# darrenjkt/SEE-VCN

Measured on AMD Instinct MI355X. Metric: scenes/sec (VCN+voxel+spconv fwd+bwd), higher is better.
Workload: dtype f32; 1 GPU; VCN_VC fwd on 64 objects x 1024 pts -> kNN surface select (k=30) -> largest DBSCAN cluster (eps 0.4) -> unique + replace (<0.1 m) into 16 KITTI-shaped 64-beam scenes (21.0k pts in range each) -> DynMeanVFE -> VoxelBackBone8x + HeightCompression fwd+bwd + SGD (BASELINE configs[1]+[2]); scenes_per_gpu=16, objects_per_gpu=64, points_per_object=1024, geometry=KITTI [0,-40,-3,70.4,40,1] @ [0.05,0.05,0.1] -> sparse [41,1600,1408], parallelism=dp1, input_side=side stream, one batch ahead (every step = 1 front + 1 compute)

## Files before the change

### see-vcn_amd/csrc/norm.h

```cpp
#pragma once
#include "common.h"

#define BN_THREADS 256
#define BN_MAX_C 512
#define BN_MAX_WGS 1024

struct BnArgs {
  const float* x;
  const float* dy;
  float* out;
  const float* gamma;
  const float* beta;
  float* running_mean;
  float* running_var;
  float* save_mean;
  float* save_invstd;
  float* dgamma;
  float* dbeta;
  float* partial;
  float* coef;
  int64_t n;
  int C, relu, wgs;
  float momentum, eps;
  int64_t* num_batches_tracked;
};

__device__ __forceinline__ float bn_shift(float mean, float scale, float beta) { return __fmaf_rn(-mean, scale, beta); }
__device__ __forceinline__ float bn_act(float x, float scale, float shift) { return __fmaf_rn(x, scale, shift); }

void sv_bn_finalize_fwd(const BnArgs& a, hipStream_t st);
void sv_bn_finalize_bwd(const BnArgs& a, hipStream_t st);
```

### see-vcn_amd/csrc/norm.hip

```cpp
#include <string.h>

#include "common.h"

#include "norm.h"

template <bool BWD>
__global__ __launch_bounds__(BN_THREADS) void k_bn_reduce(BnArgs a) {
  __shared__ float s_red[2][BN_THREADS * 4];
  const int tid = threadIdx.x, C4 = a.C >> 2;
  const int R = BN_THREADS / C4;
  const int c4 = tid % C4, rr = tid / C4;
  const bool active = rr < R;
  const int64_t rows_per_wg = (a.n + a.wgs - 1) / a.wgs;
  const int64_t r0 = (int64_t)blockIdx.x * rows_per_wg, r1 = min(a.n, r0 + rows_per_wg);
  float4 s0 = make_float4(0, 0, 0, 0), s1 = make_float4(0, 0, 0, 0);
  float4 mean = make_float4(0, 0, 0, 0), istd = mean, g = make_float4(1, 1, 1, 1), bt = mean;
  if (BWD && active) {
    mean = reinterpret_cast<const float4*>(a.save_mean)[c4], istd = reinterpret_cast<const float4*>(a.save_invstd)[c4];
    if (a.gamma) g = reinterpret_cast<const float4*>(a.gamma)[c4];
    if (a.beta) bt = reinterpret_cast<const float4*>(a.beta)[c4];
  }
  const float4 sc = make_float4(istd.x * g.x, istd.y * g.y, istd.z * g.z, istd.w * g.w);
  const float4 sh = make_float4(bn_shift(mean.x, sc.x, bt.x), bn_shift(mean.y, sc.y, bt.y), bn_shift(mean.z, sc.z, bt.z), bn_shift(mean.w, sc.w, bt.w));
  if (active) {
    for (int64_t r = r0 + rr; r < r1; r += R) {
      const float4 v = reinterpret_cast<const float4*>(a.x + r * a.C)[c4];
      if (!BWD) {
        s0.x += v.x, s0.y += v.y, s0.z += v.z, s0.w += v.w;
        s1.x += v.x * v.x, s1.y += v.y * v.y, s1.z += v.z * v.z, s1.w += v.w * v.w;
      } else {
        float4 d = reinterpret_cast<const float4*>(a.dy + r * a.C)[c4];
        const float4 xh = make_float4((v.x - mean.x) * istd.x, (v.y - mean.y) * istd.y, (v.z - mean.z) * istd.z, (v.w - mean.w) * istd.w);
        if (a.relu) {
          d.x = (bn_act(v.x, sc.x, sh.x) > 0.f) ? d.x : 0.f, d.y = (bn_act(v.y, sc.y, sh.y) > 0.f) ? d.y : 0.f;
          d.z = (bn_act(v.z, sc.z, sh.z) > 0.f) ? d.z : 0.f, d.w = (bn_act(v.w, sc.w, sh.w) > 0.f) ? d.w : 0.f;
        }
        s0.x += d.x, s0.y += d.y, s0.z += d.z, s0.w += d.w;
        s1.x += d.x * xh.x, s1.y += d.y * xh.y, s1.z += d.z * xh.z, s1.w += d.w * xh.w;
      }
    }
  }
  reinterpret_cast<float4*>(s_red[0])[tid] = s0;
  reinterpret_cast<float4*>(s_red[1])[tid] = s1;
  __syncthreads();
  if (tid < C4) {
    float4 t0 = make_float4(0, 0, 0, 0), t1 = t0;
    for (int q = 0; q < R; ++q) {
      const float4 u0 = reinterpret_cast<float4*>(s_red[0])[q * C4 + tid], u1 = reinterpret_cast<float4*>(s_red[1])[q * C4 + tid];
      t0.x += u0.x, t0.y += u0.y, t0.z += u0.z, t0.w += u0.w;
      t1.x += u1.x, t1.y += u1.y, t1.z += u1.z, t1.w += u1.w;
    }
    float* p = a.partial + (size_t)blockIdx.x * 2 * a.C;
    reinterpret_cast<float4*>(p)[tid] = t0;
    reinterpret_cast<float4*>(p + a.C)[tid] = t1;
  }
}

__device__ __forceinline__ void bn_combine(const BnArgs& a, int c, double* s0, double* s1, double& t0, double& t1) {
  const int tid = threadIdx.x;
  t0 = 0.0, t1 = 0.0;
  for (int w = tid; w < a.wgs; w += BN_THREADS) {
    t0 += (double)a.partial[(size_t)w * 2 * a.C + c];
    t1 += (double)a.partial[(size_t)w * 2 * a.C + a.C + c];
  }
  s0[tid] = t0, s1[tid] = t1;
  __syncthreads();
  for (int off = BN_THREADS / 2; off > 0; off >>= 1) {
    if (tid < off) s0[tid] += s0[tid + off], s1[tid] += s1[tid + off];
    __syncthreads();
  }
  t0 = s0[0], t1 = s1[0];
}
__device__ __forceinline__ void bn_finish_fwd(const BnArgs& a, int c, double t0, double t1, double n) {
  const float gm = a.gamma ? a.gamma[c] : 1.f, bb = a.beta ? a.beta[c] : 0.f;
  const double m = t0 / n;
  double var = t1 / n - m * m;
  var = var < 0.0 ? 0.0 : var;
  const float invstd = (float)(1.0 / sqrt(var + (double)a.eps));
  a.save_mean[c] = (float)m, a.save_invstd[c] = invstd;
  if (a.running_mean) {
    const double unbiased = n > 1.0 ? var * n / (n - 1.0) : var;
    a.running_mean[c] = (1.f - a.momentum) * a.running_mean[c] + a.momentum * (float)m;
    a.running_var[c] = (1.f - a.momentum) * a.running_var[c] + a.momentum * (float)unbiased;
  }
  const float scale = invstd * gm;
  a.coef[c] = scale;
  a.coef[a.C + c] = bn_shift((float)m, scale, bb);
}
__device__ __forceinline__ void bn_coef_bwd(const BnArgs& a, int c, double t0, double t1, double n) {
  const float gm = a.gamma ? a.gamma[c] : 1.f;
  const float invstd = a.save_invstd[c], m = a.save_mean[c];
  a.coef[c] = gm * invstd;
  a.coef[a.C + c] = (float)(t0 / n);
  a.coef[2 * a.C + c] = (float)(t1 / n);
  a.coef[3 * a.C + c] = m;
}

template <bool BWD>
__global__ __launch_bounds__(BN_THREADS) void k_bn_finalize(BnArgs a) {
  __shared__ double s0[BN_THREADS], s1[BN_THREADS];
  const int c = blockIdx.x;
  if (!BWD && c == 0 && threadIdx.x == 0 && a.num_batches_tracked) *a.num_batches_tracked += 1;
  double t0, t1;
  bn_combine(a, c, s0, s1, t0, t1);
  if (threadIdx.x != 0) return;
  if (!BWD) {
    bn_finish_fwd(a, c, t0, t1, (double)a.n);
  } else {
    a.dbeta[c] = (float)t0, a.dgamma[c] = (float)t1;
    bn_coef_bwd(a, c, t0, t1, (double)a.n);
  }
}

template <bool BWD>
__global__ __launch_bounds__(BN_THREADS) void k_bn_sums_local(BnArgs a, double* out) {
  __shared__ double s0[BN_THREADS], s1[BN_THREADS];
  const int c = blockIdx.x;
  double t0, t1;
  bn_combine(a, c, s0, s1, t0, t1);
  if (threadIdx.x != 0) return;
  out[c] = t0, out[a.C + c] = t1;
  if (!BWD && c == 0) out[2 * a.C] = (double)a.n;
  if (BWD) a.dbeta[c] = (float)t0, a.dgamma[c] = (float)t1;
}
// ... 5 lines not shown
  for (int r = 1; r < world; ++r) t0 += gathered[r * stride + c], t1 += gathered[r * stride + a.C + c], n += gathered[r * stride + 2 * a.C];
  if (c == 0) {
    if (a.num_batches_tracked) *a.num_batches_tracked += 1;
    if (total_rows) *total_rows = n;
  }
  bn_finish_fwd(a, c, t0, t1, n);
}
__global__ void k_bn_coef_bwd_global(BnArgs a, const double* gathered, int world, const double* total_rows) {
  const int c = blockIdx.x * blockDim.x + threadIdx.x;
  if (c >= a.C) return;
  const size_t stride = 2 * (size_t)a.C;
  double t0 = gathered[c], t1 = gathered[a.C + c];
  for (int r = 1; r < world; ++r) t0 += gathered[r * stride + c], t1 += gathered[r * stride + a.C + c];
  bn_coef_bwd(a, c, t0, t1, *total_rows);
}

__global__ __launch_bounds__(BN_THREADS) void k_bn_apply_fwd(BnArgs a) {
  const int C4 = a.C >> 2;
  const int64_t total = a.n * C4;
  for (int64_t i = (int64_t)blockIdx.x * BN_THREADS + threadIdx.x; i < total; i += (int64_t)gridDim.x * BN_THREADS) {
    const int c4 = (int)(i % C4);
    const float4 v = reinterpret_cast<const float4*>(a.x)[i];
    const float4 sc = reinterpret_cast<const float4*>(a.coef)[c4], sh = reinterpret_cast<const float4*>(a.coef + a.C)[c4];
    float4 y = make_float4(bn_act(v.x, sc.x, sh.x), bn_act(v.y, sc.y, sh.y), bn_act(v.z, sc.z, sh.z), bn_act(v.w, sc.w, sh.w));
    if (a.relu) y.x = fmaxf(y.x, 0.f), y.y = fmaxf(y.y, 0.f), y.z = fmaxf(y.z, 0.f), y.w = fmaxf(y.w, 0.f);
    reinterpret_cast<float4*>(a.out)[i] = y;
  }
}

__global__ __launch_bounds__(BN_THREADS) void k_bn_apply_bwd(BnArgs a) {
  const int C4 = a.C >> 2;
  const int64_t total = a.n * C4;
  for (int64_t i = (int64_t)blockIdx.x * BN_THREADS + threadIdx.x; i < total; i += (int64_t)gridDim.x * BN_THREADS) {
    const int c4 = (int)(i % C4);
    const float4 v = reinterpret_cast<const float4*>(a.x)[i];
    float4 d = reinterpret_cast<const float4*>(a.dy)[i];
    const float4 k = reinterpret_cast<const float4*>(a.coef)[c4], md = reinterpret_cast<const float4*>(a.coef + a.C)[c4];
    const float4 mx = reinterpret_cast<const float4*>(a.coef + 2 * a.C)[c4], m = reinterpret_cast<const float4*>(a.coef + 3 * a.C)[c4];
    const float4 istd = reinterpret_cast<const float4*>(a.save_invstd)[c4];
    const float4 xh = make_float4((v.x - m.x) * istd.x, (v.y - m.y) * istd.y, (v.z - m.z) * istd.z, (v.w - m.w) * istd.w);
    if (a.relu) {
      const float4 g = a.gamma ? reinterpret_cast<const float4*>(a.gamma)[c4] : make_float4(1, 1, 1, 1);
      const float4 bt = a.beta ? reinterpret_cast<const float4*>(a.beta)[c4] : make_float4(0, 0, 0, 0);
      const float4 sc = make_float4(istd.x * g.x, istd.y * g.y, istd.z * g.z, istd.w * g.w);
      const float4 sh = make_float4(bn_shift(m.x, sc.x, bt.x), bn_shift(m.y, sc.y, bt.y), bn_shift(m.z, sc.z, bt.z), bn_shift(m.w, sc.w, bt.w));
      d.x = (bn_act(v.x, sc.x, sh.x) > 0.f) ? d.x : 0.f, d.y = (bn_act(v.y, sc.y, sh.y) > 0.f) ? d.y : 0.f;
      d.z = (bn_act(v.z, sc.z, sh.z) > 0.f) ? d.z : 0.f, d.w = (bn_act(v.w, sc.w, sh.w) > 0.f) ? d.w : 0.f;
    }
    reinterpret_cast<float4*>(a.out)[i] = make_float4(k.x * (d.x - md.x - xh.x * mx.x), k.y * (d.y - md.y - xh.y * mx.y),
                                                      k.z * (d.z - md.z - xh.z * mx.z), k.w * (d.w - md.w - xh.w * mx.w));
  }
}

constexpr int BNF_THREADS = 1024;
__global__ __launch_bounds__(BNF_THREADS) void k_bn_bwd_fused(BnArgs a) {
  __shared__ double s_sum[BNF_THREADS * 4];
  __shared__ __attribute__((aligned(16))) float s_coef[4 * BN_MAX_C];
  const int tid = threadIdx.x, C = a.C, C2 = 2 * C, Q = C2 / 4, G = BNF_THREADS / Q;
  {
    const int q = tid % Q, g = tid / Q;
    double t0 = 0.0, t1 = 0.0, t2 = 0.0, t3 = 0.0;
    if (g < G) {
      for (int w = g; w < a.wgs; w += G) {
        const float4 v = reinterpret_cast<const float4*>(a.partial + (size_t)w * C2)[q];
        t0 += (double)v.x, t1 += (double)v.y, t2 += (double)v.z, t3 += (double)v.w;
      }
      double* d = s_sum + (size_t)g * C2 + 4 * q;
      d[0] = t0, d[1] = t1, d[2] = t2, d[3] = t3;
    }
  }
  __syncthreads();
  if (tid < C) {
    double t0 = 0.0, t1 = 0.0;
    for (int g = 0; g < G; ++g) t0 += s_sum[(size_t)g * C2 + tid], t1 += s_sum[(size_t)g * C2 + C + tid];
    const float gm = a.gamma ? a.gamma[tid] : 1.f;
    const float invstd = a.save_invstd[tid], m = a.save_mean[tid];
    if (blockIdx.x == 0) a.dbeta[tid] = (float)t0, a.dgamma[tid] = (float)t1;
    s_coef[tid] = gm * invstd;
    s_coef[C + tid] = (float)(t0 / (double)a.n);
    s_coef[2 * C + tid] = (float)(t1 / (double)a.n);
    s_coef[3 * C + tid] = m;
  }
  __syncthreads();
  const int C4 = C >> 2;
  const int64_t total = a.n * C4;
  for (int64_t i = (int64_t)blockIdx.x * BNF_THREADS + tid; i < total; i += (int64_t)gridDim.x * BNF_THREADS) {
    const int c4 = (int)(i % C4);
    const float4 v = reinterpret_cast<const float4*>(a.x)[i];
    float4 d = reinterpret_cast<const float4*>(a.dy)[i];
    const float4 k = reinterpret_cast<const float4*>(s_coef)[c4], md = reinterpret_cast<const float4*>(s_coef + C)[c4];
    const float4 mx = reinterpret_cast<const float4*>(s_coef + 2 * C)[c4], m = reinterpret_cast<const float4*>(s_coef + 3 * C)[c4];
    const float4 istd = reinterpret_cast<const float4*>(a.save_invstd)[c4];
    const float4 xh = make_float4((v.x - m.x) * istd.x, (v.y - m.y) * istd.y, (v.z - m.z) * istd.z, (v.w - m.w) * istd.w);
    if (a.relu) {
      const float4 g = a.gamma ? reinterpret_cast<const float4*>(a.gamma)[c4] : make_float4(1, 1, 1, 1);
      const float4 bt = a.beta ? reinterpret_cast<const float4*>(a.beta)[c4] : make_float4(0, 0, 0, 0);
      const float4 sc = make_float4(istd.x * g.x, istd.y * g.y, istd.z * g.z, istd.w * g.w);
      const float4 sh = make_float4(bn_shift(m.x, sc.x, bt.x), bn_shift(m.y, sc.y, bt.y), bn_shift(m.z, sc.z, bt.z), bn_shift(m.w, sc.w, bt.w));
      d.x = (bn_act(v.x, sc.x, sh.x) > 0.f) ? d.x : 0.f, d.y = (bn_act(v.y, sc.y, sh.y) > 0.f) ? d.y : 0.f;
      d.z = (bn_act(v.z, sc.z, sh.z) > 0.f) ? d.z : 0.f, d.w = (bn_act(v.w, sc.w, sh.w) > 0.f) ? d.w : 0.f;
    }
    reinterpret_cast<float4*>(a.out)[i] = make_float4(k.x * (d.x - md.x - xh.x * mx.x), k.y * (d.y - md.y - xh.y * mx.y),
                                                      k.z * (d.z - md.z - xh.z * mx.z), k.w * (d.w - md.w - xh.w * mx.w));
  }
}
static void bn_backward_tail(const BnArgs& a, hipStream_t st) {
  static const int fused = getenv("SEEVCN_BN_BWD_FUSED") ? atoi(getenv("SEEVCN_BN_BWD_FUSED")) : 0;
  const int Q = a.C / 2;
  if (fused && Q >= 1 && BNF_THREADS % Q == 0) {
    const int64_t quads = a.n * (a.C / 4);
    int wgs = (int)((quads + BNF_THREADS * 4 - 1) / (BNF_THREADS * 4));
    if (wgs > 256) wgs = 256;
    if (wgs < 1) wgs = 1;
    hipLaunchKernelGGL(k_bn_bwd_fused, dim3(wgs), dim3(BNF_THREADS), 0, st, a);
    return;
  }
  hipLaunchKernelGGL(k_bn_finalize<true>, dim3(a.C), dim3(BN_THREADS), 0, st, a);
  hipLaunchKernelGGL(k_bn_apply_bwd, dim3(sv_grid_1d(a.n * (a.C / 4), BN_THREADS)), dim3(BN_THREADS), 0, st, a);
}

__device__ __forceinline__ void bn_eval_coef(const float* gamma, const float* beta, const float* running_mean, const float* running_var, float eps,
                                             float* coef, int C, int c) {
  const float invstd = 1.f / sqrtf(running_var[c] + eps);
  const float gm = gamma ? gamma[c] : 1.f, bb = beta ? beta[c] : 0.f;
  coef[c] = invstd * gm;
  coef[C + c] = bb - running_mean[c] * invstd * gm;
}

__global__ void k_bn_eval_coef(BnArgs a) {
  const int c = blockIdx.x * blockDim.x + threadIdx.x;
  if (c >= a.C) return;
  bn_eval_coef(a.gamma, a.beta, a.running_mean, a.running_var, a.eps, a.coef, a.C, c);
}

struct BnEvalCoefJob {
  const float *gamma, *beta, *running_mean, *running_var;
  float* coef;
  int C;
  float eps;
};
constexpr int BN_EVAL_JOBS = 64;
struct BnEvalCoefBatch {
  BnEvalCoefJob j[BN_EVAL_JOBS];
};
static_assert(sizeof(BnEvalCoefBatch) <= 3900, "kernel argument block");

__global__ __launch_bounds__(128) void k_bn_eval_coef_batch(BnEvalCoefBatch b) {
  const BnEvalCoefJob& J = b.j[blockIdx.x];
  for (int c = threadIdx.x; c < J.C; c += 128) bn_eval_coef(J.gamma, J.beta, J.running_mean, J.running_var, J.eps, J.coef, J.C, c);
}

extern "C" int sv_batchnorm_eval_coef_batch(const int64_t* jobs_host, int n_jobs, void* stream) {
  SV_CHECK_ARG(n_jobs >= 0 && (jobs_host || n_jobs == 0), "sv_batchnorm_eval_coef_batch: bad arguments");
  if (n_jobs == 0) return SV_OK;
  for (int q = 0; q < n_jobs; ++q) {
    const int64_t* r = jobs_host + 8 * (size_t)q;
    SV_CHECK_ARG(r[2] && r[3] && r[4], "sv_batchnorm_eval_coef_batch: job %d: null pointer", q);
    SV_CHECK_ARG(r[5] >= 1 && r[5] <= BN_MAX_C, "sv_batchnorm_eval_coef_batch: job %d: 1..%d channels (got %lld)", q, BN_MAX_C, (long long)r[5]);
    SV_CHECK_ARG((uintptr_t)r[4] % 16 == 0, "sv_batchnorm_eval_coef_batch: job %d: coef_out must be 16-byte aligned", q);
  }
  hipStream_t st = sv_stream(stream);
  for (int q0 = 0; q0 < n_jobs; q0 += BN_EVAL_JOBS) {
    BnEvalCoefBatch b;
    const int nb = n_jobs - q0 < BN_EVAL_JOBS ? n_jobs - q0 : BN_EVAL_JOBS;
    for (int q = 0; q < nb; ++q) {
      const int64_t* r = jobs_host + 8 * (size_t)(q0 + q);
      BnEvalCoefJob& J = b.j[q];
      J.gamma = reinterpret_cast<const float*>((uintptr_t)r[0]), J.beta = reinterpret_cast<const float*>((uintptr_t)r[1]);
      J.running_mean = reinterpret_cast<const float*>((uintptr_t)r[2]), J.running_var = reinterpret_cast<const float*>((uintptr_t)r[3]);
      J.coef = reinterpret_cast<float*>((uintptr_t)r[4]);
      double eps;
      memcpy(&eps, &r[6], sizeof eps);
      J.C = (int)r[5], J.eps = (float)eps;
    }
    hipLaunchKernelGGL(k_bn_eval_coef_batch, dim3(nb), dim3(128), 0, st, b);
  }
  SV_LAUNCH_CHECK();
  return SV_OK;
}

static int bn_wgs(int64_t n, int C) {
  const int R = BN_THREADS / (C / 4);
  int64_t w = (n + (int64_t)R * 8 - 1) / ((int64_t)R * 8);
  if (w < 1) w = 1;
  if (w > BN_MAX_WGS) w = BN_MAX_WGS;
  return (int)w;
}

extern "C" size_t sv_batchnorm_scratch_bytes(int channels) {
  return ((size_t)BN_MAX_WGS * 2 * channels + 4 * (size_t)channels) * sizeof(float);
}

static int bn_common_check(const char* who, int64_t n, int C) {
  SV_CHECK_ARG(n >= 1, "%s: needs at least one row (got %ld)", who, (long)n);
  SV_CHECK_ARG(C >= 4 && C <= BN_MAX_C && (C & 3) == 0 && BN_THREADS % (C / 4) == 0,
               "%s: channels must be a multiple of 4 with C/4 dividing %d, <= %d (got %d)", who, BN_THREADS, BN_MAX_C, C);
  return SV_OK;
}

static void bn_scratch(BnArgs& a, void* scratch) {
  a.coef = reinterpret_cast<float*>(scratch);
  a.partial = a.coef + 4 * (size_t)a.C;
}

extern "C" int sv_batchnorm_relu_forward(const float* x, int64_t n, int channels, const float* gamma, const float* beta,
                                         float* running_mean, float* running_var, float momentum, float eps, int training, int relu,
                                         void* scratch, float* y, float* save_mean, float* save_invstd, int64_t* num_batches_tracked,
                                         void* stream) {
  if (int rc = bn_common_check("sv_batchnorm_relu_forward", n, channels)) return rc;
  SV_CHECK_ARG(x && y && scratch, "sv_batchnorm_relu_forward: null pointer");
  SV_CHECK_ARG(training ? (save_mean && save_invstd) : (running_mean && running_var),
               "sv_batchnorm_relu_forward: training needs save_mean/save_invstd, eval needs running statistics");
  BnArgs a{};
  a.x = x, a.out = y, a.gamma = gamma, a.beta = beta, a.running_mean = running_mean, a.running_var = running_var;
  a.save_mean = save_mean, a.save_invstd = save_invstd, a.n = n, a.C = channels, a.relu = relu, a.momentum = momentum, a.eps = eps;
  a.wgs = bn_wgs(n, channels);
  a.num_batches_tracked = training ? num_batches_tracked : nullptr;
  bn_scratch(a, scratch);
  hipStream_t st = sv_stream(stream);
  if (training) {
    hipLaunchKernelGGL(k_bn_reduce<false>, dim3(a.wgs), dim3(BN_THREADS), 0, st, a);
    hipLaunchKernelGGL(k_bn_finalize<false>, dim3(channels), dim3(BN_THREADS), 0, st, a);
  } else
    hipLaunchKernelGGL(k_bn_eval_coef, dim3(sv_div_up(channels, 128)), dim3(128), 0, st, a);
  hipLaunchKernelGGL(k_bn_apply_fwd, dim3(sv_grid_1d(n * (channels / 4), BN_THREADS)), dim3(BN_THREADS), 0, st, a);
  SV_LAUNCH_CHECK();
  return SV_OK;
}

extern "C" int sv_batchnorm_relu_forward_partial(const float* x, int64_t n, int channels, const float* gamma, const float* beta, float* running_mean,
                                                 float* running_var, float momentum, float eps, int relu, void* scratch, int n_partials, float* y,
                                                 float* save_mean, float* save_invstd, int64_t* num_batches_tracked, void* stream) {
  if (int rc = bn_common_check("sv_batchnorm_relu_forward_partial", n, channels)) return rc;
  SV_CHECK_ARG(x && y && scratch && save_mean && save_invstd, "sv_batchnorm_relu_forward_partial: null pointer");
  SV_CHECK_ARG(n_partials >= 1 && n_partials <= BN_MAX_WGS, "sv_batchnorm_relu_forward_partial: 1..%d partials (got %d)", BN_MAX_WGS, n_partials);
  BnArgs a{};
  a.x = x, a.out = y, a.gamma = gamma, a.beta = beta, a.running_mean = running_mean, a.running_var = running_var;
  a.save_mean = save_mean, a.save_invstd = save_invstd, a.n = n, a.C = channels, a.relu = relu, a.momentum = momentum, a.eps = eps;
  a.wgs = n_partials;
  a.num_batches_tracked = num_batches_tracked;
  bn_scratch(a, scratch);
  hipStream_t st = sv_stream(stream);
  hipLaunchKernelGGL(k_bn_finalize<false>, dim3(channels), dim3(BN_THREADS), 0, st, a);
// ... 144 lines not shown
```

### see-vcn_amd/csrc/set_abstraction_train.hip

```cpp
#include "norm.h"

typedef float st_f4 __attribute__((ext_vector_type(4)));

constexpr int ST_THREADS = 512;
constexpr int ST_WAVES = ST_THREADS / 64;
constexpr int ST_MAXC = 64;
constexpr int ST_NT = ST_MAXC / 16;
constexpr int ST_MAXF = 128;

constexpr int ST_PITCH = ST_MAXC + 4;
constexpr int ST_GRID = 512;

struct SaT {
  const float* xyz;
  const float* feat;
  const float* new_xyz;
  const int32_t* idx;
  const int32_t* row_start;
  const float* w1;
  const float* w2;
  float* z1;
  float* z2;
  float* dy1;
  float* part;
// ... 7 lines not shown
  float* zmin;
  uint8_t* amax;
  uint8_t* amin;
  float* out;
  const float* dout;
  float* wpart;
  float* S;
  float* P;
  int64_t M, N;
  int C, Kp, C1, C2, ns;
};

__device__ __forceinline__ st_f4 mfma4(const st_f4 a, const st_f4 b, st_f4 c) {
  c = __builtin_amdgcn_mfma_f32_16x16x4f32(a.x, b.x, c, 0, 0, 0);
  c = __builtin_amdgcn_mfma_f32_16x16x4f32(a.y, b.y, c, 0, 0, 0);
  c = __builtin_amdgcn_mfma_f32_16x16x4f32(a.z, b.z, c, 0, 0, 0);
  c = __builtin_amdgcn_mfma_f32_16x16x4f32(a.w, b.w, c, 0, 0, 0);
  return c;
}

__device__ __forceinline__ void tile_to_global(const float* T, float* dst, int C, int lane) {
  const int c4n = C >> 2, nf = 16 * c4n;
  for (int f = lane; f < nf; f += 64) {
    const int row = f / c4n, c4 = f - row * c4n;
    reinterpret_cast<st_f4*>(dst)[f] = *reinterpret_cast<const st_f4*>(T + row * ST_PITCH + c4 * 4);
  }
}

__device__ __forceinline__ void acc_to_lds(float* T, const st_f4 (&acc)[ST_NT], int nt, int li, int kk) {
#pragma unroll
  for (int t = 0; t < ST_NT; ++t)
    if (t < nt) {
#pragma unroll
      for (int r = 0; r < 4; ++r) T[(kk * 4 + r) * ST_PITCH + t * 16 + li] = acc[t][r];
    }
}

__device__ __forceinline__ void stats_to_partial(float (&s0)[ST_NT], float (&s1)[ST_NT], int nt, int C, float (*s_red)[2][ST_MAXC], float* part, int wid,
                                                 int lane) {
  const int li = lane & 15, kk = lane >> 4;
#pragma unroll
  for (int t = 0; t < ST_NT; ++t)
    if (t < nt) {
      float a = s0[t], b = s1[t];
      a += __shfl_xor(a, 16), b += __shfl_xor(b, 16);
      a += __shfl_xor(a, 32), b += __shfl_xor(b, 32);
      if (kk == 0) s_red[wid][0][t * 16 + li] = a, s_red[wid][1][t * 16 + li] = b;
    }
  __syncthreads();
  for (int e = threadIdx.x; e < 2 * C; e += ST_THREADS) {
    const int which = e / C, c = e - which * C;
    float v = 0.f;
    for (int w = 0; w < ST_WAVES; ++w) v += s_red[w][which][c];
    part[(size_t)blockIdx.x * 2 * C + which * C + c] = v;
  }
}

constexpr int SP_THREADS = 256;
__global__ __launch_bounds__(SP_THREADS) void k_sa_point_proj(SaT a) {
  __shared__ __attribute__((aligned(16))) float s_w[ST_MAXC * (ST_MAXF + 4)];
  __shared__ __attribute__((aligned(16))) float s_t[SP_THREADS / 64][16 * ST_PITCH];
  const int tid = threadIdx.x, lane = tid & 63, wid = tid >> 6, li = lane & 15, kk = lane >> 4;
  const int pw = a.C + 4, cin = a.C + 3;
  for (int e = tid; e < a.C1 * a.C; e += SP_THREADS) s_w[(e / a.C) * pw + e % a.C] = a.w1[(e / a.C) * cin + 3 + e % a.C];
  __syncthreads();
  float* T = s_t[wid];
  const int nt1 = a.C1 / 16, nqf = a.C / 16;
  const int64_t ntiles = (a.N + 15) / 16;
  for (int64_t tile = (int64_t)blockIdx.x * (SP_THREADS / 64) + wid; tile < ntiles; tile += (int64_t)gridDim.x * (SP_THREADS / 64)) {
    const int64_t n = tile * 16 + li;
    st_f4 acc[ST_NT];
#pragma unroll
    for (int t = 0; t < ST_NT; ++t) acc[t] = (st_f4){0.f, 0.f, 0.f, 0.f};
    for (int qs = 0; qs < nqf; ++qs) {
      st_f4 A = (st_f4){0.f, 0.f, 0.f, 0.f};
      if (n < a.N) A = *reinterpret_cast<const st_f4*>(a.feat + n * a.C + qs * 16 + kk * 4);
#pragma unroll
      for (int t = 0; t < ST_NT; ++t)
        if (t < nt1) acc[t] = mfma4(A, *reinterpret_cast<const st_f4*>(s_w + (t * 16 + li) * pw + qs * 16 + kk * 4), acc[t]);
    }
    acc_to_lds(T, acc, nt1, li, kk);
    __builtin_amdgcn_fence(__ATOMIC_RELEASE, "wavefront");
    const int rows = (int)min((int64_t)16, a.N - tile * 16);
    const int c4n = a.C1 >> 2;
    for (int f = lane; f < rows * c4n; f += 64) {
      const int row = f / c4n, c4 = f - row * c4n;
      reinterpret_cast<st_f4*>(a.P + tile * 16 * a.C1)[f] = *reinterpret_cast<const st_f4*>(T + row * ST_PITCH + c4 * 4);
    }
    __builtin_amdgcn_fence(__ATOMIC_RELEASE, "wavefront");
  }
}

constexpr int SG_THREADS = 256;
template <int NT1, int NT2>
__global__ __launch_bounds__(SG_THREADS) void k_sa_fwd1(SaT a_in) {
  SaT a = a_in;
  if (NT1) a.C1 = NT1 * 16;
  if (NT2) a.C2 = NT2 * 16;
  __shared__ __attribute__((aligned(16))) float s_wx[3][ST_MAXC];
  __shared__ float s_red[SG_THREADS / 64][2][ST_MAXC];
  const int tid = threadIdx.x, lane = tid & 63, wid = tid >> 6, li = lane & 15, kk = lane >> 4;
  for (int e = tid; e < 3 * ST_MAXC; e += SG_THREADS) s_wx[e / ST_MAXC][e % ST_MAXC] = (e % ST_MAXC) < a.C1 ? a.w1[(e % ST_MAXC) * (a.C + 3) + e / ST_MAXC] : 0.f;
  __syncthreads();
  const int nt1 = NT1 ? NT1 : a.C1 / 16, G = a.ns / 16;
  st_f4 s0[ST_NT], s1[ST_NT];
#pragma unroll
  for (int qs = 0; qs < ST_NT; ++qs) s0[qs] = s1[qs] = (st_f4){0.f, 0.f, 0.f, 0.f};
  for (int64_t q = (int64_t)blockIdx.x * (SG_THREADS / 64) + wid; q < a.M; q += (int64_t)gridDim.x * (SG_THREADS / 64)) {
    const bool empty = a.idx[q * a.ns] < 0;
    const int64_t base = a.row_start[q];
    const float qx = a.new_xyz[q * 3], qy = a.new_xyz[q * 3 + 1], qz = a.new_xyz[q * 3 + 2];
    for (int g = 0; g < G; ++g) {
      const int64_t row = q * a.ns + g * 16 + li;
      float dx = 0.f, dy = 0.f, dz = 0.f;
      int64_t src = -1;
      if (!empty) {
        src = base + a.idx[row];
        const float* p = a.xyz + src * 3;
        dx = p[0] - qx, dy = p[1] - qy, dz = p[2] - qz;
      }
#pragma unroll
      for (int qs = 0; qs < ST_NT; ++qs)
        if (qs < nt1) {
          const int c = qs * 16 + kk * 4;
          st_f4 z = (st_f4){0.f, 0.f, 0.f, 0.f};
          if (!empty) {
            if (a.P) z = *reinterpret_cast<const st_f4*>(a.P + src * a.C1 + c);
            const st_f4 wx = *reinterpret_cast<const st_f4*>(s_wx[0] + c), wy = *reinterpret_cast<const st_f4*>(s_wx[1] + c),
                        wz = *reinterpret_cast<const st_f4*>(s_wx[2] + c);
#pragma unroll
            for (int i = 0; i < 4; ++i) z[i] = fmaf(wz[i], dz, fmaf(wy[i], dy, fmaf(wx[i], dx, z[i])));
          }
          *reinterpret_cast<st_f4*>(a.z1 + row * a.C1 + c) = z;
#pragma unroll
          for (int i = 0; i < 4; ++i) s0[qs][i] += z[i], s1[qs][i] += z[i] * z[i];
        }
    }
  }
#pragma unroll
  for (int qs = 0; qs < ST_NT; ++qs)
    if (qs < nt1) {
#pragma unroll
      for (int i = 0; i < 4; ++i) {
        float u = s0[qs][i], v = s1[qs][i];
#pragma unroll
        for (int off = 1; off < 16; off <<= 1) u += __shfl_xor(u, off), v += __shfl_xor(v, off);
        if (li == 0) s_red[wid][0][qs * 16 + kk * 4 + i] = u, s_red[wid][1][qs * 16 + kk * 4 + i] = v;
      }
    }
  __syncthreads();
  for (int e = tid; e < 2 * a.C1; e += SG_THREADS) {
    const int which = e / a.C1, c = e - which * a.C1;
    float v = 0.f;
    for (int w = 0; w < SG_THREADS / 64; ++w) v += s_red[w][which][c];
    a.part[(size_t)blockIdx.x * 2 * a.C1 + which * a.C1 + c] = v;
  }
}

template <int NT1, int NT2>
__global__ __launch_bounds__(ST_THREADS, 4) void k_sa_fwd2(SaT a_in) {
  SaT a = a_in;
  if (NT1) a.C1 = NT1 * 16;
  if (NT2) a.C2 = NT2 * 16;
  __shared__ __attribute__((aligned(16))) float s_w2[ST_MAXC * (ST_MAXC + 4)];
  __shared__ __attribute__((aligned(16))) float s_t[ST_WAVES][16 * ST_PITCH];
  __shared__ float s_red[ST_WAVES][2][ST_MAXC];
  const int tid = threadIdx.x, lane = tid & 63, wid = tid >> 6, li = lane & 15, kk = lane >> 4;
  __shared__ __attribute__((aligned(16))) float s_c1[2][ST_MAXC];
  const int p2 = a.C1 + 4;
  for (int e = tid; e < a.C2 * a.C1; e += ST_THREADS) s_w2[(e / a.C1) * p2 + e % a.C1] = a.w2[e];
  for (int e = tid; e < a.C1; e += ST_THREADS) s_c1[0][e] = a.coef1[e], s_c1[1][e] = a.coef1[a.C1 + e];
  __syncthreads();
  float* T = s_t[wid];
  const int nt1 = NT1 ? NT1 : a.C1 / 16, nt2 = NT2 ? NT2 : a.C2 / 16, G = a.ns / 16;
  float s0[ST_NT] = {0.f, 0.f, 0.f, 0.f}, s1[ST_NT] = {0.f, 0.f, 0.f, 0.f};
  for (int64_t q = (int64_t)blockIdx.x * ST_WAVES + wid; q < a.M; q += (int64_t)gridDim.x * ST_WAVES) {
    float vmax[ST_NT], vmin[ST_NT];
    int smax[ST_NT], smin[ST_NT];
#pragma unroll
    for (int t = 0; t < ST_NT; ++t) vmax[t] = -3.4e38f, vmin[t] = 3.4e38f, smax[t] = smin[t] = 0;
    for (int g = 0; g < G; ++g) {
      const int64_t rowbase = q * a.ns + g * 16;
      st_f4 acc[ST_NT];
#pragma unroll
      for (int t = 0; t < ST_NT; ++t) acc[t] = (st_f4){0.f, 0.f, 0.f, 0.f};
      st_f4 Az[ST_NT];
#pragma unroll
      for (int qs = 0; qs < ST_NT; ++qs) {
        Az[qs] = (st_f4){0.f, 0.f, 0.f, 0.f};
        if (qs < nt1) Az[qs] = *reinterpret_cast<const st_f4*>(a.z1 + (rowbase + li) * a.C1 + qs * 16 + kk * 4);
      }
#pragma unroll
      for (int qs = 0; qs < ST_NT; ++qs)
        if (qs < nt1) {
          const st_f4 sc = *reinterpret_cast<const st_f4*>(s_c1[0] + qs * 16 + kk * 4), sh = *reinterpret_cast<const st_f4*>(s_c1[1] + qs * 16 + kk * 4);
          st_f4 A = Az[qs];
          A.x = fmaxf(fmaf(A.x, sc.x, sh.x), 0.f), A.y = fmaxf(fmaf(A.y, sc.y, sh.y), 0.f);
          A.z = fmaxf(fmaf(A.z, sc.z, sh.z), 0.f), A.w = fmaxf(fmaf(A.w, sc.w, sh.w), 0.f);
#pragma unroll
          for (int t = 0; t < ST_NT; ++t)
            if (t < nt2) acc[t] = mfma4(A, *reinterpret_cast<const st_f4*>(s_w2 + (t * 16 + li) * p2 + qs * 16 + kk * 4), acc[t]);
        }
#pragma unroll
      for (int t = 0; t < ST_NT; ++t)
#pragma unroll
        for (int r = 0; r < 4; ++r) {
          const float v = acc[t][r];
          const int slot = g * 16 + kk * 4 + r;
// ... 11 lines not shown
      if (t < nt2) {
#pragma unroll
        for (int off = 16; off < 64; off <<= 1) {
          const float ov = __shfl_xor(vmax[t], off), ow = __shfl_xor(vmin[t], off);
          const int os = __shfl_xor(smax[t], off), ot = __shfl_xor(smin[t], off);
          if (ov > vmax[t] || (ov == vmax[t] && os < smax[t])) vmax[t] = ov, smax[t] = os;
          if (ow < vmin[t] || (ow == vmin[t] && ot < smin[t])) vmin[t] = ow, smin[t] = ot;
        }
        if (kk == 0) {
          const int64_t o = q * a.C2 + t * 16 + li;
          a.zmax[o] = vmax[t], a.zmin[o] = vmin[t], a.amax[o] = (uint8_t)smax[t], a.amin[o] = (uint8_t)smin[t];
        }
      }
  }
  stats_to_partial(s0, s1, nt2, a.C2, s_red, a.part, wid, lane);
}

__global__ __launch_bounds__(256) void k_sa_out(SaT a) {
  const int64_t total = a.M * a.C2;
  for (int64_t i = (int64_t)blockIdx.x * 256 + threadIdx.x; i < total; i += (int64_t)gridDim.x * 256) {
    const int c = (int)(i % a.C2);
    const float sc = a.coef2[c], sh = a.coef2[a.C2 + c];
    const bool pos = sc >= 0.f;
    const float sel = pos ? a.zmax[i] : a.zmin[i];
    a.out[i] = fmaxf(fmaf(sel, sc, sh), 0.f);
    a.zmax[i] = sel;
    a.amax[i] = pos ? a.amax[i] : a.amin[i];
  }
}

__global__ __launch_bounds__(256) void k_sa_bwd0(SaT a) {
  __shared__ float s_r[2][256];
  const int tid = threadIdx.x, C = a.C2;
  const int rpw = 256 / C;
  const int c = tid % C, rr = tid / C;
  const bool active = rr < rpw;
  const int64_t rows_per_wg = (a.M + gridDim.x - 1) / gridDim.x;
  const int64_t r0 = (int64_t)blockIdx.x * rows_per_wg, r1 = min(a.M, r0 + rows_per_wg);
  float t0 = 0.f, t1 = 0.f;
  if (active) {
    const float m = a.mean2[c], is = a.istd2[c];
    for (int64_t r = r0 + rr; r < r1; r += rpw) {
      const int64_t i = r * C + c;
      const float d = a.out[i] > 0.f ? a.dout[i] : 0.f;
      a.zmin[i] = d;
      t0 += d, t1 += d * ((a.zmax[i] - m) * is);
    }
  }
  s_r[0][tid] = active ? t0 : 0.f, s_r[1][tid] = active ? t1 : 0.f;
  __syncthreads();
  if (tid < C) {
    float u0 = 0.f, u1 = 0.f;
    for (int k = 0; k < rpw; ++k) u0 += s_r[0][k * C + tid], u1 += s_r[1][k * C + tid];
    a.part[(size_t)blockIdx.x * 2 * C + tid] = u0;
    a.part[(size_t)blockIdx.x * 2 * C + C + tid] = u1;
  }
}

constexpr int ST_NTH = ST_NT / 2;
template <int NT1, int NT2>
__global__ __launch_bounds__(ST_THREADS, 4) void k_sa_bwd2(SaT a_in) {
  SaT a = a_in;
  if (NT1) a.C1 = NT1 * 16;
  if (NT2) a.C2 = NT2 * 16;
  __shared__ __attribute__((aligned(16))) float s_w2t[ST_MAXC * (ST_MAXC + 4)];
  __shared__ __attribute__((aligned(16))) float s_t[ST_WAVES][16 * ST_PITCH];
  __shared__ float s_red[ST_WAVES][2][ST_MAXC];
  const int tid = threadIdx.x, lane = tid & 63, wid = tid >> 6, li = lane & 15, kk = lane >> 4;
  const int pair = wid & 3, half = wid >> 2;
  const int pT = a.C2 + 4;
  for (int e = tid; e < a.C2 * a.C1; e += ST_THREADS) s_w2t[(e % a.C1) * pT + e / a.C1] = a.w2[e];
  __syncthreads();
  float* T = s_t[wid];
  const int nt1 = NT1 ? NT1 : a.C1 / 16, nt2 = NT2 ? NT2 : a.C2 / 16, G = a.ns / 16;
  const int u0 = half ? (nt1 + 1) / 2 : 0, u1 = half ? nt1 : (nt1 + 1) / 2;
  __shared__ float s_k[7][ST_MAXC];
  for (int c = tid; c < ST_MAXC; c += ST_THREADS) {
    float k = 0.f, A = 0.f, B = 0.f, s1v = 0.f, h1 = 0.f, i1 = 0.f, n1 = 0.f;
    if (c < a.C2) {
      const float md = a.coef2[a.C2 + c], mx = a.coef2[2 * a.C2 + c], m = a.coef2[3 * a.C2 + c], is = a.istd2[c];
      k = a.coef2[c], A = -k * mx * is, B = k * (mx * is * m - md);
    }
    if (c < a.C1) s1v = a.coef1[c], h1 = a.coef1[a.C1 + c], i1 = a.istd1[c], n1 = -a.mean1[c] * a.istd1[c];
    s_k[0][c] = k, s_k[1][c] = A, s_k[2][c] = B, s_k[3][c] = s1v, s_k[4][c] = h1, s_k[5][c] = i1, s_k[6][c] = n1;
  }
  __syncthreads();
  st_f4 accw[ST_NT][ST_NTH];
#pragma unroll
  for (int t = 0; t < ST_NT; ++t)
#pragma unroll
    for (int j = 0; j < ST_NTH; ++j) accw[t][j] = (st_f4){0.f, 0.f, 0.f, 0.f};
  float sd[ST_NTH] = {0.f, 0.f}, sdx[ST_NTH] = {0.f, 0.f};
  for (int64_t q = (int64_t)blockIdx.x * 4 + pair; q < a.M; q += (int64_t)gridDim.x * 4) {
    float dq[ST_NT];
    int aq[ST_NT];
#pragma unroll
    for (int t = 0; t < ST_NT; ++t) {
      dq[t] = 0.f, aq[t] = -1;
      if (t < nt2) dq[t] = a.zmin[q * a.C2 + t * 16 + li], aq[t] = a.amax[q * a.C2 + t * 16 + li];
    }
    for (int g = 0; g < G; ++g) {
      const int64_t rowbase = q * a.ns + g * 16;
      st_f4 dz2[ST_NT];
#pragma unroll
      for (int t = 0; t < ST_NT; ++t) {
        dz2[t] = (st_f4){0.f, 0.f, 0.f, 0.f};
        if (t < nt2) {
#pragma unroll
// ... 427 lines not shown
```

### see-vcn_amd/csrc/sparse_conv.hip

```cpp
#include <stdlib.h>

#include "common.h"
#include "norm.h"


typedef float f32x4 __attribute__((ext_vector_type(4)));
typedef float f32x2 __attribute__((ext_vector_type(2)));
typedef int i32x4 __attribute__((ext_vector_type(4)));

struct InNorm {
  const float* coef = nullptr;
  int relu = 0;
};
static thread_local InNorm g_next_in;
extern "C" int sv_conv_next_input_norm(const float* coef, int relu) {
  g_next_in.coef = coef, g_next_in.relu = relu ? 1 : 0;
  return SV_OK;
}
static InNorm take_input_norm() {
  const InNorm r = g_next_in;
  g_next_in = InNorm{};
  return r;
}

// ... 1500 lines not shown
    for (int g = 0; g < RS_G; ++g) {
      __builtin_amdgcn_fence(__ATOMIC_RELEASE, "wavefront");
#pragma unroll
      for (int t = 0; t < NT; ++t)
#pragma unroll
        for (int r = 0; r < 4; ++r) {
          T[(kk_e * 4 + r) * TP + t * 16 + li_e] = acc[g][t][r];
        }
      __builtin_amdgcn_fence(__ATOMIC_RELEASE, "wavefront");
#pragma unroll
      for (int i = 0; i < (16 * C4N + 63) / 64; ++i) {
        const int f = lane_e + 64 * i, rw = f / C4N, c4 = f % C4N;
        if (16 * C4N % 64 == 0 || f < 16 * C4N) {
          const int64_t row = s_idx[RS3_KMAX][g * 16 + rw];
          if (row >= 0) {
            const int col = col_tile0 * 16 + c4 * 4;
            f32x4 v = *reinterpret_cast<const f32x4*>(T + rw * TP + c4 * 4);
            if (a.bias) v += *reinterpret_cast<const f32x4*>(a.bias + col);
            if (a.scale) {
              const f32x4 sc = *reinterpret_cast<const f32x4*>(a.scale + col), sh = *reinterpret_cast<const f32x4*>(a.shift + col);
              v = (f32x4){bn_act(v[0], sc[0], sh[0]), bn_act(v[1], sc[1], sh[1]), bn_act(v[2], sc[2], sh[2]), bn_act(v[3], sc[3], sh[3])};
            }
            if (a.residual) v += *reinterpret_cast<const f32x4*>(a.residual + row * pv.nc_total + col);
            if (a.relu) v = (f32x4){fmaxf(v[0], 0.f), fmaxf(v[1], 0.f), fmaxf(v[2], 0.f), fmaxf(v[3], 0.f)};
            *reinterpret_cast<f32x4*>(a.Y + row * pv.nc_total + col) = v;
          }
        }
      }
    }
    __builtin_amdgcn_fence(__ATOMIC_RELEASE, "wavefront");
  } else {
#pragma unroll
    for (int g = 0; g < RS_G; ++g)
#pragma unroll
      for (int r = 0; r < 4; ++r) {
        const int64_t row = s_idx[RS3_KMAX][g * 16 + kk_e * 4 + r];
        if (row < 0) continue;
#pragma unroll
        for (int t = 0; t < NT; ++t) {
          const int col = (col_tile0 + t) * 16 + li_e;
          a.Y[row * pv.nc_total + col] = conv_epilogue(acc[g][t][r], col, row, a);
        }
      }
  }
    if (DBG && pv.trace) t_mark = __builtin_amdgcn_s_memtime();
  }
  if (pv.bn_partial) {
    if constexpr (DYN) {
      __syncthreads();
      for (int e = threadIdx.x; e < 2 * NT * 16; e += 256) {
        const int which = e / (NT * 16), c = e % (NT * 16);
        float v = 0.f;
        for (int pos = 0; pos < dyn_n; ++pos) v += s_bnpos[which][pos * (NT * 16) + c];
        pv.bn_partial[((size_t)blockIdx.x * 2 + which) * pv.nc_total + col_tile0 * 16 + c] = v;
      }
    } else {
    __shared__ float s_bn[4][2][64];
    if (NT == 4 || lane < NT * 16) s_bn[wid][0][lane] = bn0, s_bn[wid][1][lane] = bn1;
    __syncthreads();
    for (int e = threadIdx.x; e < 2 * NT * 16; e += 256) {
      const int which = e / (NT * 16), c = e % (NT * 16);
      const float v = (s_bn[0][which][c] + s_bn[1][which][c]) + (s_bn[2][which][c] + s_bn[3][which][c]);
      pv.bn_partial[((size_t)blockIdx.x * 2 + which) * pv.nc_total + col_tile0 * 16 + c] = v;
    }
    }
  }
  if (DBG && pv.trace && lane == 0) {
    asm volatile("s_waitcnt vmcnt(0)" ::: "memory");
    const unsigned long long t_end = __builtin_amdgcn_s_memtime();
    unsigned hw = 0, xcc = 0;
    asm volatile("s_getreg_b32 %0, hwreg(HW_REG_HW_ID)" : "=s"(hw));
    asm volatile("s_getreg_b32 %0, hwreg(HW_REG_XCC_ID)" : "=s"(xcc));
    const unsigned work = trace_work;
    unsigned long long* o = pv.trace + (((size_t)blockIdx.y * gridDim.x + blockIdx.x) * 4 + wid) * 8;
    o[0] = t_start, o[1] = t_pro, o[2] = t_loop, o[3] = t_end, o[4] = hw, o[5] = xcc, o[6] = work, o[7] = ((unsigned long long)blockIdx.x << 8) | wid;
  }
}

static bool rs3_applies(int K, int Kd, int Nc) {
  if (K > RS3_KMAX || K < 1) return false;
  const bool kd_ok = Kd == 16 || Kd == 32 || Kd == 64 || Kd == 128;
  const bool nc_ok = Nc == 16 || Nc == 32 || (Nc >= 64 && Nc % 64 == 0 && Nc <= 512);
  return kd_ok && nc_ok;
}
extern "C" int sv_conv_planned_partials(void) { return PL_REGIONS * PL_REGION_WAVES / 4; }

extern "C" int sv_conv_mfma_kernel_applies(int K, int Kd, int Nc, int64_t n_src) {
  return (rs3_applies(K, Kd, Nc) && (uint64_t)(n_src < 0 ? 0 : n_src) * Kd * 4 < 0xfffffff0ull) ? 1 : 0;
}

template <int NT, int KQ>
static void launch_rs3_g(const ConvArgs& a, const PlanView& pv, const float* wfrag, uint32_t xb, uint32_t wb, dim3 grid, hipStream_t st) {
  if (pv.debug) {
    if constexpr (NT == 4) {
      if (pv.d.G == 1) hipLaunchKernelGGL((k_spconv_rs3<NT, KQ, 1, 1>), grid, dim3(256), 0, st, a, pv, wfrag, xb, wb);
      else hipLaunchKernelGGL((k_spconv_rs3<NT, KQ, 2, 1>), grid, dim3(256), 0, st, a, pv, wfrag, xb, wb);
    } else {
      hipLaunchKernelGGL((k_spconv_rs3<NT, KQ, 4, 1>), grid, dim3(256), 0, st, a, pv, wfrag, xb, wb);
    }
    return;
  }
  if (pv.trace) {
    if constexpr (NT == 4) {
      if (pv.d.G == 1) hipLaunchKernelGGL((k_spconv_rs3<NT, KQ, 1, 2>), grid, dim3(256), 0, st, a, pv, wfrag, xb, wb);
      else hipLaunchKernelGGL((k_spconv_rs3<NT, KQ, 2, 2>), grid, dim3(256), 0, st, a, pv, wfrag, xb, wb);
    } else {
      hipLaunchKernelGGL((k_spconv_rs3<NT, KQ, 4, 2>), grid, dim3(256), 0, st, a, pv, wfrag, xb, wb);
    }
    return;
  }
  if constexpr (NT == 4) {
    static const int dyn_env = getenv("SEEVCN_RS3_DYN") ? atoi(getenv("SEEVCN_RS3_DYN")) : 0;
    if (dyn_env && 4 * pv.d.n_pass * pv.d.G * NT * 16 <= RS3_DYN_COLS) {
      if (pv.in_coef) hipLaunchKernelGGL((k_spconv_rs3<NT, KQ, 1, 0, true, true>), grid, dim3(256), 0, st, a, pv, wfrag, xb, wb);
      else hipLaunchKernelGGL((k_spconv_rs3<NT, KQ, 1, 0, false, true>), grid, dim3(256), 0, st, a, pv, wfrag, xb, wb);
      return;
// ... 1268 lines not shown
```

Before: 4528 scenes/sec.

## Transpose BN partial sums to channel-major layout with wave-shuffle final reduction

BatchNorm partial sums change from workgroup-major ([wg][2][C]) to channel-major ([2][C][pitch]), so each per-channel finalize block reads its partials contiguously instead of striding by 2*C. The producers in sparse conv, set-abstraction training and the BN reduce kernel all switch to the new indexing. The last tree-reduction steps in bn_combine use wave shuffles instead of shared memory and barriers, and the unused env-gated fused BN backward kernel is removed. In exchange, producers now write scattered to global memory, which may cost more on the write side, and the layout requires every producer to pass a consistent wgs (gridDim.x), or the reads will be misaligned.

```diff
diff --git a/see-vcn_amd/csrc/norm.h b/see-vcn_amd/csrc/norm.h
--- a/see-vcn_amd/csrc/norm.h
+++ b/see-vcn_amd/csrc/norm.h
@@ -28,5 +28,8 @@
 __device__ __forceinline__ float bn_shift(float mean, float scale, float beta) { return __fmaf_rn(-mean, scale, beta); }
 __device__ __forceinline__ float bn_act(float x, float scale, float shift) { return __fmaf_rn(x, scale, shift); }
 
+__host__ __device__ __forceinline__ int bn_pitch(int wgs) { return (wgs + 31) & ~31; }
+__device__ __forceinline__ size_t bn_partial_at(int which, int c, int C, int wgs, int w) { return ((size_t)which * C + c) * bn_pitch(wgs) + w; }
+
 void sv_bn_finalize_fwd(const BnArgs& a, hipStream_t st);
 void sv_bn_finalize_bwd(const BnArgs& a, hipStream_t st);
diff --git a/see-vcn_amd/csrc/norm.hip b/see-vcn_amd/csrc/norm.hip
--- a/see-vcn_amd/csrc/norm.hip
+++ b/see-vcn_amd/csrc/norm.hip
@@ -50,26 +50,31 @@
       t0.x += u0.x, t0.y += u0.y, t0.z += u0.z, t0.w += u0.w;
       t1.x += u1.x, t1.y += u1.y, t1.z += u1.z, t1.w += u1.w;
     }
-    float* p = a.partial + (size_t)blockIdx.x * 2 * a.C;
-    reinterpret_cast<float4*>(p)[tid] = t0;
-    reinterpret_cast<float4*>(p + a.C)[tid] = t1;
+    float* p0 = a.partial + bn_partial_at(0, 4 * tid, a.C, a.wgs, blockIdx.x), *p1 = a.partial + bn_partial_at(1, 4 * tid, a.C, a.wgs, blockIdx.x);
+    const int pitch = bn_pitch(a.wgs);
+    p0[0] = t0.x, p0[pitch] = t0.y, p0[2 * pitch] = t0.z, p0[3 * pitch] = t0.w;
+    p1[0] = t1.x, p1[pitch] = t1.y, p1[2 * pitch] = t1.z, p1[3 * pitch] = t1.w;
   }
 }
 
 __device__ __forceinline__ void bn_combine(const BnArgs& a, int c, double* s0, double* s1, double& t0, double& t1) {
   const int tid = threadIdx.x;
+  const float* p0 = a.partial + bn_partial_at(0, c, a.C, a.wgs, 0), *p1 = a.partial + bn_partial_at(1, c, a.C, a.wgs, 0);
   t0 = 0.0, t1 = 0.0;
   for (int w = tid; w < a.wgs; w += BN_THREADS) {
-    t0 += (double)a.partial[(size_t)w * 2 * a.C + c];
-    t1 += (double)a.partial[(size_t)w * 2 * a.C + a.C + c];
+    t0 += (double)p0[w];
+    t1 += (double)p1[w];
   }
   s0[tid] = t0, s1[tid] = t1;
   __syncthreads();
-  for (int off = BN_THREADS / 2; off > 0; off >>= 1) {
+  for (int off = BN_THREADS / 2; off >= 64; off >>= 1) {
     if (tid < off) s0[tid] += s0[tid + off], s1[tid] += s1[tid + off];
     __syncthreads();
   }
-  t0 = s0[0], t1 = s1[0];
+  if (tid < 64) {
+    t0 = s0[tid], t1 = s1[tid];
+    for (int off = 32; off > 0; off >>= 1) t0 += __shfl_down(t0, off), t1 += __shfl_down(t1, off);
+  }
 }
 __device__ __forceinline__ void bn_finish_fwd(const BnArgs& a, int c, double t0, double t1, double n) {
   const float gm = a.gamma ? a.gamma[c] : 1.f, bb = a.beta ? a.beta[c] : 0.f;
@@ -181,69 +186,7 @@
   }
 }
 
-constexpr int BNF_THREADS = 1024;
-__global__ __launch_bounds__(BNF_THREADS) void k_bn_bwd_fused(BnArgs a) {
-  __shared__ double s_sum[BNF_THREADS * 4];
-  __shared__ __attribute__((aligned(16))) float s_coef[4 * BN_MAX_C];
-  const int tid = threadIdx.x, C = a.C, C2 = 2 * C, Q = C2 / 4, G = BNF_THREADS / Q;
-  {
-    const int q = tid % Q, g = tid / Q;
-    double t0 = 0.0, t1 = 0.0, t2 = 0.0, t3 = 0.0;
-    if (g < G) {
-      for (int w = g; w < a.wgs; w += G) {
-        const float4 v = reinterpret_cast<const float4*>(a.partial + (size_t)w * C2)[q];
-        t0 += (double)v.x, t1 += (double)v.y, t2 += (double)v.z, t3 += (double)v.w;
-      }
-      double* d = s_sum + (size_t)g * C2 + 4 * q;
-      d[0] = t0, d[1] = t1, d[2] = t2, d[3] = t3;
-    }
-  }
-  __syncthreads();
-  if (tid < C) {
-    double t0 = 0.0, t1 = 0.0;
-    for (int g = 0; g < G; ++g) t0 += s_sum[(size_t)g * C2 + tid], t1 += s_sum[(size_t)g * C2 + C + tid];
-    const float gm = a.gamma ? a.gamma[tid] : 1.f;
-    const float invstd = a.save_invstd[tid], m = a.save_mean[tid];
-    if (blockIdx.x == 0) a.dbeta[tid] = (float)t0, a.dgamma[tid] = (float)t1;
-    s_coef[tid] = gm * invstd;
-    s_coef[C + tid] = (float)(t0 / (double)a.n);
-    s_coef[2 * C + tid] = (float)(t1 / (double)a.n);
-    s_coef[3 * C + tid] = m;
-  }
-  __syncthreads();
-  const int C4 = C >> 2;
-  const int64_t total = a.n * C4;
-  for (int64_t i = (int64_t)blockIdx.x * BNF_THREADS + tid; i < total; i += (int64_t)gridDim.x * BNF_THREADS) {
-    const int c4 = (int)(i % C4);
-    const float4 v = reinterpret_cast<const float4*>(a.x)[i];
-    float4 d = reinterpret_cast<const float4*>(a.dy)[i];
-    const float4 k = reinterpret_cast<const float4*>(s_coef)[c4], md = reinterpret_cast<const float4*>(s_coef + C)[c4];
-    const float4 mx = reinterpret_cast<const float4*>(s_coef + 2 * C)[c4], m = reinterpret_cast<const float4*>(s_coef + 3 * C)[c4];
-    const float4 istd = reinterpret_cast<const float4*>(a.save_invstd)[c4];
-    const float4 xh = make_float4((v.x - m.x) * istd.x, (v.y - m.y) * istd.y, (v.z - m.z) * istd.z, (v.w - m.w) * istd.w);
-    if (a.relu) {
-      const float4 g = a.gamma ? reinterpret_cast<const float4*>(a.gamma)[c4] : make_float4(1, 1, 1, 1);
-      const float4 bt = a.beta ? reinterpret_cast<const float4*>(a.beta)[c4] : make_float4(0, 0, 0, 0);
-      const float4 sc = make_float4(istd.x * g.x, istd.y * g.y, istd.z * g.z, istd.w * g.w);
-      const float4 sh = make_float4(bn_shift(m.x, sc.x, bt.x), bn_shift(m.y, sc.y, bt.y), bn_shift(m.z, sc.z, bt.z), bn_shift(m.w, sc.w, bt.w));
-      d.x = (bn_act(v.x, sc.x, sh.x) > 0.f) ? d.x : 0.f, d.y = (bn_act(v.y, sc.y, sh.y) > 0.f) ? d.y : 0.f;
-      d.z = (bn_act(v.z, sc.z, sh.z) > 0.f) ? d.z : 0.f, d.w = (bn_act(v.w, sc.w, sh.w) > 0.f) ? d.w : 0.f;
-    }
-    reinterpret_cast<float4*>(a.out)[i] = make_float4(k.x * (d.x - md.x - xh.x * mx.x), k.y * (d.y - md.y - xh.y * mx.y),
-                                                      k.z * (d.z - md.z - xh.z * mx.z), k.w * (d.w - md.w - xh.w * mx.w));
-  }
-}
 static void bn_backward_tail(const BnArgs& a, hipStream_t st) {
-  static const int fused = getenv("SEEVCN_BN_BWD_FUSED") ? atoi(getenv("SEEVCN_BN_BWD_FUSED")) : 0;
-  const int Q = a.C / 2;
-  if (fused && Q >= 1 && BNF_THREADS % Q == 0) {
-    const int64_t quads = a.n * (a.C / 4);
-    int wgs = (int)((quads + BNF_THREADS * 4 - 1) / (BNF_THREADS * 4));
-    if (wgs > 256) wgs = 256;
-    if (wgs < 1) wgs = 1;
-    hipLaunchKernelGGL(k_bn_bwd_fused, dim3(wgs), dim3(BNF_THREADS), 0, st, a);
-    return;
-  }
   hipLaunchKernelGGL(k_bn_finalize<true>, dim3(a.C), dim3(BN_THREADS), 0, st, a);
   hipLaunchKernelGGL(k_bn_apply_bwd, dim3(sv_grid_1d(a.n * (a.C / 4), BN_THREADS)), dim3(BN_THREADS), 0, st, a);
 }
@@ -317,7 +260,7 @@
 }
 
 extern "C" size_t sv_batchnorm_scratch_bytes(int channels) {
-  return ((size_t)BN_MAX_WGS * 2 * channels + 4 * (size_t)channels) * sizeof(float);
+  return ((size_t)2 * channels * bn_pitch(BN_MAX_WGS) + 4 * (size_t)channels) * sizeof(float);
 }
 
 static int bn_common_check(const char* who, int64_t n, int C) {
diff --git a/see-vcn_amd/csrc/set_abstraction_train.hip b/see-vcn_amd/csrc/set_abstraction_train.hip
--- a/see-vcn_amd/csrc/set_abstraction_train.hip
+++ b/see-vcn_amd/csrc/set_abstraction_train.hip
@@ -83,7 +83,7 @@
     const int which = e / C, c = e - which * C;
     float v = 0.f;
     for (int w = 0; w < ST_WAVES; ++w) v += s_red[w][which][c];
-    part[(size_t)blockIdx.x * 2 * C + which * C + c] = v;
+    part[bn_partial_at(which, c, C, gridDim.x, blockIdx.x)] = v;
   }
 }
 
@@ -184,7 +184,7 @@
     const int which = e / a.C1, c = e - which * a.C1;
     float v = 0.f;
     for (int w = 0; w < SG_THREADS / 64; ++w) v += s_red[w][which][c];
-    a.part[(size_t)blockIdx.x * 2 * a.C1 + which * a.C1 + c] = v;
+    a.part[bn_partial_at(which, c, a.C1, gridDim.x, blockIdx.x)] = v;
   }
 }
 
@@ -302,8 +302,8 @@
   if (tid < C) {
     float u0 = 0.f, u1 = 0.f;
     for (int k = 0; k < rpw; ++k) u0 += s_r[0][k * C + tid], u1 += s_r[1][k * C + tid];
-    a.part[(size_t)blockIdx.x * 2 * C + tid] = u0;
-    a.part[(size_t)blockIdx.x * 2 * C + C + tid] = u1;
+    a.part[bn_partial_at(0, tid, C, gridDim.x, blockIdx.x)] = u0;
+    a.part[bn_partial_at(1, tid, C, gridDim.x, blockIdx.x)] = u1;
   }
 }
 
diff --git a/see-vcn_amd/csrc/sparse_conv.hip b/see-vcn_amd/csrc/sparse_conv.hip
--- a/see-vcn_amd/csrc/sparse_conv.hip
+++ b/see-vcn_amd/csrc/sparse_conv.hip
@@ -1576,7 +1576,7 @@
         const int which = e / (NT * 16), c = e % (NT * 16);
         float v = 0.f;
         for (int pos = 0; pos < dyn_n; ++pos) v += s_bnpos[which][pos * (NT * 16) + c];
-        pv.bn_partial[((size_t)blockIdx.x * 2 + which) * pv.nc_total + col_tile0 * 16 + c] = v;
+        pv.bn_partial[bn_partial_at(which, col_tile0 * 16 + c, pv.nc_total, gridDim.x, blockIdx.x)] = v;
       }
     } else {
     __shared__ float s_bn[4][2][64];
@@ -1585,7 +1585,7 @@
     for (int e = threadIdx.x; e < 2 * NT * 16; e += 256) {
       const int which = e / (NT * 16), c = e % (NT * 16);
       const float v = (s_bn[0][which][c] + s_bn[1][which][c]) + (s_bn[2][which][c] + s_bn[3][which][c]);
-      pv.bn_partial[((size_t)blockIdx.x * 2 + which) * pv.nc_total + col_tile0 * 16 + c] = v;
+      pv.bn_partial[bn_partial_at(which, col_tile0 * 16 + c, pv.nc_total, gridDim.x, blockIdx.x)] = v;
     }
     }
   }
```

New measurement: 4528 scenes/sec. No clear change (-0.0%).
